# EI-CoreBioinformatics/portcullis

Measured on AMD Instinct MI355X. Metric: junc_reads_per_sec, higher is better.
Workload: dtype int32; 1 GPU; BASELINE configs[2]: synthetic 199999998 paired-end 150-bp reads, 25 contigs of GRCh38 lengths (3088286401 bp), 249999 junctions, orientation FR; reads_total=199999998, junctions_total=249999, contigs=25, reads_rank0=199999998, pairs_rank0=66692850

## Files before the change

### portcullis_amd/csrc/pjb_api.hip

```cpp
#include "pjb_host.hip.h"
#include "pjb_kernels.hip.h"

static int slot_init(pjb_ctx *c, int k);
static void aux_streams(pjb_ctx *c) {
    if (!c->stream3) (void)hipStreamCreateWithFlags(&c->stream3, hipStreamNonBlocking);
    if (!c->stream4) (void)hipStreamCreateWithFlags(&c->stream4, hipStreamNonBlocking);
}

extern "C" {

namespace {
std::mutex g_host_mu;
std::map<void *, size_t> g_host_registered;
}
void *pjb_host_alloc(size_t bytes) {
    if (bytes >= ((size_t)8 << 20)) {
        const size_t huge = (size_t)2 << 20, len = (bytes + huge - 1) & ~(huge - 1);
        void *p = mmap(nullptr, len, PROT_READ | PROT_WRITE, MAP_PRIVATE | MAP_ANONYMOUS, -1, 0);
        if (p != MAP_FAILED) {
            (void)madvise(p, len, MADV_HUGEPAGE);
            const size_t nt = std::min<size_t>(4, len >> 24);
            auto touch = [&](size_t t) {
                const size_t per = ((len / std::max<size_t>(nt, 1)) + huge - 1) & ~(huge - 1), a = std::min(len, per * t), b = std::min(len, a + per);
                for (size_t o = a; o < b; o += 4096) ((volatile uint8_t *)p)[o] = 0;
// ... 85 lines not shown
    hipDeviceProp_t prop;
    e = hipGetDeviceProperties(&prop, cfg->device);
    if (e != hipSuccess) return fail(nullptr, PJB_ERR_HIP, "hipGetDeviceProperties: %s", hipGetErrorString(e));
    cmark("hipSetDevice, hipGetDeviceProperties");
    const int n_cu = prop.multiProcessorCount;
    if (prop.warpSize != 64)
        return fail(nullptr, PJB_ERR_NO_DEVICE, "device %d (%s) is not a wave64 CDNA device", cfg->device, prop.gcnArchName);
    pjb_ctx *c = new (std::nothrow) pjb_ctx();
    if (!c) return fail(nullptr, PJB_ERR_NOMEM, "out of host memory");
    const int dev = cfg->device;
    auto attributes = [dev] {
        (void)hipSetDevice(dev);
        ingest_kernel_attributes();
        (void)hipFuncSetAttribute((const void *)rs_scatter<0, u64>, hipFuncAttributeMaxDynamicSharedMemorySize, (int)rs_scatter_lds_bytes(RS_MAX_BITS));
        (void)hipFuncSetAttribute((const void *)rs_scatter<0, u32>, hipFuncAttributeMaxDynamicSharedMemorySize, (int)rs_scatter_lds_bytes(RS_MAX_BITS, 4));
    };
    std::thread attr_thread(attributes);
    struct JoinAttr {
        std::thread &t;
        ~JoinAttr() {
            if (t.joinable()) t.join();
        }
    } join_attr{attr_thread};
    c->cfg = *cfg;
    memset(&c->timing, 0, sizeof c->timing);
    e = hipStreamCreateWithFlags(&c->stream, hipStreamNonBlocking);
    if (e != hipSuccess) {
        delete c;
        return fail(nullptr, PJB_ERR_HIP, "hipStreamCreate: %s", hipGetErrorString(e));
    }
// ... 706 lines not shown
        pass_bits.assign((size_t)n_pass, sort_bits / n_pass);
        for (int p = 0; p < sort_bits % n_pass; p++) pass_bits[(size_t)p]++;
        const int dbits = pass_bits[0];
        int rc2;
        if ((rc2 = ensure(c, S.hist, (size_t)plan_tiles * (1u << dbits) * 4))) return rc2;
        if ((rc2 = ensure(c, S.hist_scan, (size_t)plan_tiles * (1u << dbits) * 4))) return rc2;
        if ((rc2 = ensure(c, S.bintotal, (size_t)4 << dbits))) return rc2;
        if ((rc2 = ensure(c, S.hist_part, (size_t)((plan_tiles + RSP_TILES - 1) / RSP_TILES) * (1u << dbits) * 4))) return rc2;
        return PJB_OK;
    };
    const bool run_route = lim.dense && lim.run_sort;
    RunOut ro;
    memset(&ro, 0, sizeof ro);
    const u32 run_cap = (u32)std::min<u64>((u64)PL / 8 + 64ull * rs_tiles, 0xfff00000ull);
    const u32 ro_tiles = (run_cap + RS_TILE - 1) / RS_TILE;
    u64 *ro_total = nullptr, *ro_key[2] = {nullptr, nullptr};
    u32 *run_dest = nullptr, *ro_idx[2] = {nullptr, nullptr};
    if (run_route) {
        auto al = [](size_t b) { return (b + 255) & ~(size_t)255; };
        const size_t slack = (size_t)run_cap + RS_TILE;
        const size_t at_tf = 256, at_tn = at_tf + al((size_t)rs_tiles * 4), at_key = at_tn + al((size_t)rs_tiles * 4), at_cnt = at_key + al(slack * 8),
                     at_dest = at_cnt + al((size_t)run_cap * 4), at_k0 = at_dest + al((size_t)run_cap * 4), at_k1 = at_k0 + al(slack * 8),
                     at_i0 = at_k1 + al(slack * 8), at_i1 = at_i0 + al(slack * 4), at_end = at_i1 + al(slack * 4);
        if ((rc = ensure(c, S.runs, at_end))) return rc;
        uint8_t *b = (uint8_t *)S.runs.p;
        ro.n_runs = (u32 *)b;
        ro_total = (u64 *)(b + 8);
        ro.tile_first = (u32 *)(b + at_tf);
        ro.tile_n = (u32 *)(b + at_tn);
        ro.key = (u64 *)(b + at_key);
// ... 29 lines not shown
        if (run_route) plan_tiles = ro_tiles;
        if ((rc = plan_passes())) return rc;
        LAUNCH(c, "kd_assign", kd_assign, dim3(rs_tiles), dim3(256), okey, d_P, kf, (const u64 *)S.bitmap.p, (const u32 *)S.wrank.p,
               (const u32 *)S.ends.p, (const u32 *)S.firstid.p, JL, (const u64 *)S.total.p, (u32 *)S.jidbam.p, (u32 *)S.acc.p, (const u64 *)S.jkey.p,
               (const int32_t *)S.ancl.p, (const int32_t *)S.ancr.p, d_err, d_cs, run_route ? 0 : pass_bits[0], (u32 *)S.hist.p, ro);
        first_hist_done = !run_route;
        if ((rc = fork_k4b())) return rc;
        LAUNCH(c, "kd_reset", kd_reset, dim3(cand_blocks), dim3(256), (const u64 *)cand, (const u32 *)cand_rank, kf, JL, (const ContigStats *)d_cs,
               (u64 *)S.bitmap.p, (u32 *)S.ends.p, (u32 *)S.pagecnt.p);
        S.dense_at_rest = true;
    } else if ((rc = plan_passes()))
        return rc;
    int cur = 0, shift = 0;
    static const char *const rs_names[4] = {"rs_hist", "rs_panel_sums", "rs_panel_scan", "rs_scatter"};
    static const char *const ro_names[6] = {"ro_hist", "ro_panel_sums", "ro_panel_scan", "ro_scatter", "ro_offsets", "rs_place"};
    auto sort_pass = [&](auto key_tag, const void *kin_v, void *kout_v, const u32 *vin, u32 *vout, int bits, const u32 *d_n, u32 tiles,
                         const char *const *names) -> int {
        using K = decltype(key_tag);
        const K *kin = (const K *)kin_v;
        K *kout = (K *)kout_v;
        if (!(shift == 0 && first_hist_done))
            LAUNCH(c, names[0], rs_hist<K>, dim3(tiles), dim3(256), kin, d_n, shift, bits, (u32 *)S.hist.p, tiles);
        {
            const u32 nb = 1u << bits, n_panels = (tiles + RSP_TILES - 1) / RSP_TILES;
            LAUNCH(c, names[1], rs_panel_sums, dim3(n_panels, (nb + 255) / 256), dim3(256), (const u32 *)S.hist.p, tiles, nb, (u32 *)S.hist_part.p);
            LAUNCH(c, names[2], rs_panel_scan, dim3(n_panels, (nb + 255) / 256), dim3(256), (const u32 *)S.hist.p, (const u32 *)S.hist_part.p, tiles, nb,
                   (u32 *)S.hist_scan.p, (u32 *)S.bintotal.p);
        }
#define RS_SCATTER(B)                                                                                                                          \
    LAUNCH_LDS(c, names[3], (rs_scatter<B, K>), dim3(tiles), dim3(256), rs_scatter_lds_bytes(bits, sizeof(K)), kin, vin, kout, vout, d_n, \
               shift, bits, (const u32 *)S.hist_scan.p, (const u32 *)S.bintotal.p, tiles)
        switch (bits) {
        case 9: RS_SCATTER(9); break;
        case 10: RS_SCATTER(10); break;
        case 11: RS_SCATTER(11); break;
        default: RS_SCATTER(0); break;
        }
#undef RS_SCATTER
        return PJB_OK;
    };
    for (int p = 0; p < n_pass; p++) {
        const int bits = pass_bits[(size_t)p];
        if (bits <= 0) break;
        if (run_route) {
            rc = sort_pass((u64)0, p == 0 ? (const void *)ro.key : (const void *)ro_key[cur], ro_key[cur ^ 1], p == 0 ? nullptr : (const u32 *)ro_idx[cur],
                           ro_idx[cur ^ 1], bits, (const u32 *)ro.n_runs, ro_tiles, ro_names);
        } else {
            const u32 *vin = p == 0 ? nullptr : (const u32 *)S.idx[cur].p;
            u32 *vout = (u32 *)S.idx[cur ^ 1].p;
            if (lim.dense) rc = sort_pass((u32)0, p == 0 ? S.jidbam.p : S.key[cur].p, S.key[cur ^ 1].p, vin, vout, bits, d_P, rs_tiles, rs_names);
            else rc = sort_pass((u64)0, p == 0 ? S.okey.p : S.key[cur].p, S.key[cur ^ 1].p, vin, vout, bits, d_P, rs_tiles, rs_names);
        }
        if (rc) return rc;
        cur ^= 1;
        shift += bits;
    }
    if (run_route) {
        const u32 *order = ro_idx[cur];
        if ((rc = run_scan(c, ro_names[4], RunCountFn{(const u32 *)ro.cnt, order}, RunDestSink{run_dest, order}, (u64)run_cap, ro_total, (const u32 *)ro.n_runs)))
            return rc;
        cur = 1;
        LAUNCH(c, ro_names[5], rs_place, dim3(rs_tiles), dim3(256), (const u32 *)S.jidbam.p, d_P, (const u64 *)ro.key, (const u32 *)run_dest,
               (const u32 *)ro.tile_first, (const u32 *)ro.tile_n, run_cap, ro.tile_bits, (u32 *)S.key[cur].p, (u32 *)S.idx[cur].p);
        n_pass = 1;
    }
    f.n_pass = n_pass;
    const u32 *sidx = (const u32 *)S.idx[cur].p;
    f.sidx = sidx;
    const u32 *jid_sorted = lim.dense ? (const u32 *)S.key[cur].p : (const u32 *)S.jid.p;
    f.jid_sorted = jid_sorted;
    STAGE_EVENT(2);
    if ((rc = ensure(c, S.entsum, (size_t)JL * 8 + 16))) return rc;
    const u32 n_slices_lim = (PL + 63) / 64 + 1;
    const hipStream_t tl = st;
// ... 101 lines not shown
    }
    const hipStream_t rows_stream = c->side_stream ? c->stream3 : tl;
    if (rows_stream != tl) {
        HIP_TRY(c, hipEventRecord(S.ev_rows, tl));
        HIP_TRY(c, hipStreamWaitEvent(rows_stream, S.ev_rows, 0));
    }
    {
        struct StreamScope {
            pjb_ctx *c;
            hipStream_t main;
            ~StreamScope() { c->stream = main; }
        } scope{c, c->stream};
        c->stream = rows_stream;
        LAUNCH(c, "k6_rows_out", k6_rows_out, dim3(K6_BLOCKS), dim3(256), (const u64 *)S.rows.p, (const ContigStats *)d_cs,
               (u64 *)c->rows_table, row_base, mirror_base, (RowCursor *)c->b_cursor.p, mirror_table, mirror_room, d_err, d_gen_cnt, S.pub_dev,
               (const MemberStats *)d_members, d_member_junc, n_members);
    }
    S.at_rest = true;
    HIP_TRY(c, hipEventRecord(S.ev[7], rows_stream));
    HIP_TRY(c, hipEventRecord(S.ev_done, rows_stream));
#undef STAGE_EVENT
    f.queued = true;
    return PJB_OK;
}

static void wait_flight(pjb_ctx *c, Flight &f) {
    if (f.queued) (void)hipEventSynchronize(c->sl[f.slot].ev_done);
}

static void unqueue_followers(pjb_ctx *c) {
    for (int k = 1; k < c->n_fl; k++) {
// ... 277 lines not shown
            R.n_junctions = ms[m].n_junc;
            pairs += ms[m].n_pairs;
            juncs += ms[m].n_junc;
        }
        if (pairs != cs.n_pairs || juncs != J)
            return fail(c, PJB_ERR_STATE, "finish_group: members hold %llu pairs / %llu junctions, the chain %llu / %u", (unsigned long long)pairs,
                        (unsigned long long)juncs, (unsigned long long)cs.n_pairs, J);
        Rsum.spliced = cs.spliced;
        Rsum.unspliced = cs.unspliced;
        Rsum.sum_len = cs.sum_len;
        Rsum.min_len = cs.min_len;
        Rsum.max_len = cs.max_len;
    }
    c->junc_seen = std::max(c->junc_seen, group ? J / (u32)n_members : J);
    if (f.n_reads > 0) c->junc_per_read = std::max(c->junc_per_read, (double)J / (double)f.n_reads);
    c->timing.sort_passes = f.n_pass;
    c->timing.repeats = repeats;
    c->timing.repeat_reasons = repeat_reasons;
    c->timing.generic_pairs = 0;
    c->timing.generic_reads = 0;
    c->timing.checked_reads = *(const u32 *)(S.pub + PUB_CHECKED_AT);
    for (u32 k = 0; k < GEN_SHARDS; k++) {
        c->timing.generic_pairs += ((const u32 *)(S.pub + PUB_GEN_AT))[k];
        c->timing.generic_reads += ((const u32 *)(S.pub + PUB_GREADS_AT))[k];
    }
    c->timing.position_runs = cs.R;
    c->timing.candidates = lim.dense ? cs.n_cand : 0;
    const size_t old = c->rows_n;
    {
        u32 at[2];
// ... 275 lines not shown
}

int pjb_set_option(pjb_ctx *c, const char *name, int64_t value) {
    if (!c || !name) return PJB_ERR_ARG;
    if (c->n_fl) return fail(c, PJB_ERR_STATE, "set_option: target %d is still queued", c->fl[0].tid);
    const std::string n = name;
    if (n == "overlap") c->side_stream = value != 0;
    else if (n == "dense_ids") c->dense_ids = value != 0;
    else if (n == "extra_dense") c->extra_dense_only = value != 0;
    else if (n == "sort_floor") c->sort_floor = (u32)std::max<int64_t>(1, std::min<int64_t>(value, 1 << 30));
    else if (n == "window_skip") c->window_skip = value != 0;
    else if (n == "run_sort") c->run_sort = value != 0;
    else if (n == "run_window") {
        if (value < 0 || value > (int64_t)RUN_W) return fail(c, PJB_ERR_ARG, "set_option: run_window takes 0 (the default, %u) to %u", RUN_W, RUN_W);
        c->run_window = (u32)value;
    } else if (n == "grow_batch") {
        if (value < 0 || value > 32768) return fail(c, PJB_ERR_ARG, "set_option: grow_batch takes 0 (the default: what the pool holds) to 32768 trees");
        c->grow_batch = (u32)value;
    } else if (n == "knn_chunk") {
        if (value < 0 || value > (1 << 22)) return fail(c, PJB_ERR_ARG, "set_option: knn_chunk takes 0 (the default: sized to fill the chip) to %d base rows", 1 << 22);
        c->knn_chunk = (u32)value;
    } else if (n == "list_cap") c->list_cap_forced = (u32)std::max<int64_t>(0, std::min<int64_t>(value, 1 << 30));
    else return fail(c, PJB_ERR_ARG, "set_option: unknown option '%s'", name);
    return PJB_OK;
}

int pjb_get_timing(const pjb_ctx *c, pjb_timing *out) {
    if (!c || !out) return PJB_ERR_ARG;
    if (c->cfg.abi_version >= 4) *out = c->timing;
    else memcpy(out, &c->timing, offsetof(pjb_timing, repeats));
// ... 5 lines not shown
```

### portcullis_amd/csrc/pjb_device.hip.h

```cpp
#pragma once

#include <hip/hip_runtime.h>
#include <stdint.h>

#include "../../include/portcullis_amd.h"

namespace pjb {

typedef unsigned long long u64;
typedef unsigned int u32;

struct DevBatch {
    const int32_t *pos;
    const uint16_t *flag;
    const uint8_t *mapq;
    const uint8_t *xs;
    const int32_t *l_qseq;
    const int32_t *mtid;
    const int32_t *mpos;
    const uint32_t *cig_off;
    const uint32_t *cigar;
    const uint32_t *seq_off;
    const uint8_t *seq4;
    const u64 *name_hash;
// ... 437 lines not shown
    __syncthreads();
    u64 run = s_pref[0] + s_pref[1] + s_pref[2] + s_pref[3];
    if (blockIdx.x == n_tiles - 1 && threadIdx.x == 0) *total = run + tile_sums[blockIdx.x];
    const u64 base = (u64)blockIdx.x * SCAN_TILE;
#pragma unroll
    for (int k = 0; k < 8; k++) {
        u64 i = base + (u64)k * 256 + threadIdx.x;
        u64 v = i < n ? f(i) : 0;
        u64 tot;
        u64 ex = block_escan_256<u64>(v, sm, &tot);
        if (i < n) g(i, v, run + ex);
        run += tot;
    }
}

struct ArrU32Fn {
    const u32 *a;
    __device__ u64 operator()(u64 i) const { return a[i]; }
};
struct ArrU8Fn {
    const uint8_t *a;
    __device__ u64 operator()(u64 i) const { return a[i]; }
};
struct ArrI32Fn {
    const int32_t *a;
    __device__ u64 operator()(u64 i) const { return (u64)(int64_t)a[i]; }
};
struct ExclusiveU32Sink {
    u32 *out;
    __device__ void operator()(u64 i, u64, u64 ex) const { out[i] = (u32)ex; }
// ... 70 lines not shown
    case 'W': return 'S';
    case 'X': return 'X';
    case 'Y': return 'R';
    default: return 0;
    }
}

__device__ __forceinline__ void fetch_clamp(int32_t glen, int32_t &b, int32_t &e) {
    if (e < b) b = e;
    if (b < 0) b = 0;
    else if (glen <= b) b = glen - 1;
    if (e < 0) e = 0;
    else if (glen <= e) e = glen - 1;
}

constexpr int PUB_BASE_AT = 240, PUB_ERR_AT = 256, PUB_XCNT_AT = 320 , PUB_CHECKED_AT = 384 , PUB_GEN_AT = 512, PUB_MEMBERS_AT = 1536, PUB_GREADS_AT = 3072, PUB_BYTES = 4096;
static_assert(PUB_MEMBERS_AT + GROUP_MAX * sizeof(MemberStats) <= PUB_BYTES && sizeof(MemberStats) % 8 == 0, "control block layout");

}
```

### portcullis_amd/csrc/pjb_host.hip.h

```cpp
#pragma once
#include "pjb_device.hip.h"
#include "pjb_extra_types.hip.h"

#include <algorithm>
#include <sys/mman.h>
#include <thread>
#include <chrono>
#include <cstdarg>
#include <cstdio>
#include <cstdlib>
#include <cstring>
#include <map>
#include <memory>
#include <mutex>
#include <string>
#include <thread>
#include <vector>

using namespace pjb;


inline thread_local std::string g_create_error;
inline thread_local std::string g_thread_error;
inline thread_local const void *g_thread_error_ctx = nullptr;
// ... 214 lines not shown
    std::vector<void *> graveyard;
    std::mutex grave_mu;
    size_t last_rows_n = 0;
    uint8_t *mirror = nullptr;
    size_t mirror_cap = 0;
    int64_t *mirror_hdr = nullptr;
    size_t mirror_rows = 0;
    int64_t mirror_acc[5] = {0, 0, 0, INT32_MAX, 0};
    pjb_timing timing;
    int radix_max_bits = 11;
    double junc_per_read = 0;
    u32 sort_floor = 1u << 16;
    bool window_skip = true;
    bool run_sort = true;
    u32 run_window = 0;
    u32 list_cap_forced = 0;
    bool k1_serial = true;
    hipEvent_t last_k1_ev = nullptr;
    int k1s_blocks_forced = 0;
    bool ktime = false;
    std::vector<std::string> knames;
    std::vector<int64_t> kcount;
    std::vector<double> kms;
    std::vector<std::string> ktime_only;
    Buf *scan_tiles = nullptr;
    Buf b_scan_tiles;
    Buf b_inf_comp, b_inf_out, b_inf_blocks, b_inf_status, b_inf_scratch, b_inf_bitmap;
    Buf b_dfl_in, b_dfl_sym, b_dfl_slots, b_dfl_size, b_dfl_off, b_dfl_packed;
    Buf b_bam_seg, b_bam_rec, b_bam_ctl;
    struct IndexState *index = nullptr;
// ... 239 lines not shown
    Buf &tiles = c->scan_tiles ? *c->scan_tiles : c->b_scan_tiles;
    int rc = ensure(c, tiles, (size_t)nt * 8);
    if (rc) return rc;
    u64 *ts = (u64 *)tiles.p;
    std::string t = tag;
    LAUNCH(c, (t + "_reduce").c_str(), (scan_reduce_kernel<F>), dim3(nt), dim3(256), f, n, ts, d_n);
    if (nt <= SCAN2_MAX_TILES) {
        LAUNCH(c, (t + "_apply").c_str(), (scan_apply2_kernel<F, G>), dim3(nt), dim3(256), f, g, n, (const u64 *)ts, d_n, d_total);
        return PJB_OK;
    }
    LAUNCH(c, (t + "_tiles").c_str(), scan_tiles_kernel, dim3(1), dim3(1024), ts, nt, d_total);
    LAUNCH(c, (t + "_apply").c_str(), (scan_apply_kernel<F, G>), dim3(nt), dim3(256), f, g, n, (const u64 *)ts, d_n);
    return PJB_OK;
}

inline void *slab_alloc(pjb_ctx *c, OpenContig &oc, size_t bytes) {
    bytes = (std::max<size_t>(bytes, 16) + 255) & ~(size_t)255;
    for (auto &s : oc.slabs)
        if (s.cap - s.used >= bytes) {
            void *r = s.p + s.used;
            s.used += bytes;
            return r;
        }
    {
        const size_t want = oc.slabs.empty() ? std::max(bytes, oc.slab_hint) : bytes;
        long best = -1;
        for (size_t k = 0; k < c->slab_pool.size(); k++)
            if (c->slab_pool[k].cap >= want && (best < 0 || c->slab_pool[k].cap < c->slab_pool[(size_t)best].cap)) best = (long)k;
        if (best >= 0) {
            Slab s = c->slab_pool[(size_t)best];
// ... 84 lines not shown
```

### portcullis_amd/csrc/pjb_kernels.hip.h

```cpp
#pragma once

#include "pjb_device.hip.h"

namespace pjb {

__global__ __launch_bounds__(256) void k0_upper(uint8_t *g, int64_t n, int do_upper, int *has_x) {
    int64_t i = ((int64_t)blockIdx.x * 256 + threadIdx.x) * 16;
    bool x = false;
    for (int64_t j = i; j < n && j < i + 16; j++) {
        uint8_t c = g[j];
        x |= (c == 'X' || (do_upper && c == 'x'));
    }
    if (__ballot(x) && lane_id() == 0) atomicOr(has_x, 1);
    if (!do_upper) return;
    if (i + 16 <= n && ((uintptr_t)(g + i) & 15) == 0) {
        uint4 v = *reinterpret_cast<uint4 *>(g + i);
        u32 *w = reinterpret_cast<u32 *>(&v);
#pragma unroll
        for (int k = 0; k < 4; k++) {
            u32 x = w[k], r = 0;
#pragma unroll
            for (int b = 0; b < 4; b++) {
                u32 c = (x >> (8 * b)) & 0xff;
                if (c >= 'a' && c <= 'z') c -= 32;
// ... 2152 lines not shown
__device__ __forceinline__ void wave_hist_add(u32 *h, u32 d, bool valid) {
    u64 rem = __ballot(valid);
    const int lane = lane_id();
#pragma unroll
    for (int it = 0; it < 2; it++) {
        if (rem == 0) return;
        const int first = __ffsll((long long)rem) - 1;
        const u32 d0 = __shfl(d, first, 64);
        const u64 m = __ballot(valid && d == d0) & rem;
        if (lane == first) atomicAdd(&h[d0], (u32)__popcll(m));
        rem &= ~m;
    }
    if ((rem >> lane) & 1ull) atomicAdd(&h[d], 1u);
}

template <typename K>
__global__ __launch_bounds__(256) void rs_hist(const K *keys, const u32 *np, int shift, int bits, u32 *hist, u32 n_tiles) {
    __shared__ u32 h[RS_MAX_BINS];
    const u32 n = *np;
    const u32 nb = 1u << bits;
    for (u32 d = threadIdx.x; d < nb; d += 256) h[d] = 0;
    __syncthreads();
    const u32 base = blockIdx.x * RS_TILE;
    const u32 mask = nb - 1;
    K kk[RS_ITEMS];
#pragma unroll
    for (int k = 0; k < RS_ITEMS; k++) {
        const u32 i = base + k * 256 + threadIdx.x;
        kk[k] = i < n ? keys[i] : (K)0;
    }
#pragma unroll
    for (int k = 0; k < RS_ITEMS; k++) {
        const u32 i = base + k * 256 + threadIdx.x;
        wave_hist_add(h, (u32)(kk[k] >> shift) & mask, i < n);
    }
    __syncthreads();
    for (u32 d = threadIdx.x; d < nb; d += 256) hist[(size_t)blockIdx.x * nb + d] = h[d];
}

constexpr u32 RSP_TILES = 64;
__global__ __launch_bounds__(256) void rs_panel_sums(const u32 *hist, u32 n_tiles, u32 nb, u32 *psum) {
    const u32 d = blockIdx.y * 256 + threadIdx.x;
    if (d >= nb) return;
    const u32 t0 = blockIdx.x * RSP_TILES, t1 = t0 + RSP_TILES < n_tiles ? t0 + RSP_TILES : n_tiles;
    u32 sum = 0;
    for (u32 t = t0; t < t1; t += 8) {
        u32 v[8];
#pragma unroll
        for (int k = 0; k < 8; k++) v[k] = t + k < t1 ? hist[(size_t)(t + k) * nb + d] : 0u;
#pragma unroll
        for (int k = 0; k < 8; k++) sum += v[k];
    }
// ... 11 lines not shown
#pragma unroll
        for (int k = 0; k < 8; k++) run += v[k];
    }
    const u32 t0 = panel * RSP_TILES, t1 = t0 + RSP_TILES < n_tiles ? t0 + RSP_TILES : n_tiles;
    for (u32 t = t0; t < t1; t += 8) {
        u32 v[8];
#pragma unroll
        for (int k = 0; k < 8; k++) v[k] = t + k < t1 ? hist[(size_t)(t + k) * nb + d] : 0u;
#pragma unroll
        for (int k = 0; k < 8; k++) {
            if (t + k < t1) hist_scan[(size_t)(t + k) * nb + d] = run;
            run += v[k];
        }
    }
    if (t1 == n_tiles) row_total[d] = run;
}

__host__ __device__ constexpr size_t rs_scatter_lds_bytes(int bits, size_t key_bytes = 8) {
    return (size_t)RS_TILE * key_bytes + ((size_t)4 << bits) + ((size_t)8 << bits);
}
constexpr int RS_PF = 2;

template <int BITS>
__device__ __forceinline__ u64 wave_match_digit(u32 d, bool valid, int bits) {
    u64 peers = __ballot(valid);
    u32 lo = (u32)peers, hi = (u32)(peers >> 32);
    auto step = [&](int bit) {
        const int m = __builtin_amdgcn_sbfe((int)d, bit, 1);
        const u64 bb = __ballot(m != 0);
        lo &= ~((u32)bb ^ (u32)m);
        hi &= ~((u32)(bb >> 32) ^ (u32)m);
    };
    if constexpr (BITS > 0) {
#pragma unroll
        for (int bit = 0; bit < BITS; bit++) step(bit);
    } else {
        for (int bit = 0; bit < bits; bit++) step(bit);
    }
    return ((u64)hi << 32) | lo;
}

template <int BITS, typename K>
__global__ __launch_bounds__(256, 3) void rs_scatter(const K *kin, const u32 *vin, K *kout, u32 *vout, const u32 *np, int shift,
                                                      int bits, const u32 *hist_scan, const u32 *row_total, u32 n_tiles) {
    extern __shared__ __attribute__((aligned(16))) unsigned char rs_smem[];
    __shared__ u64 s_scan[4];
    const u32 n = *np;
    if ((u64)blockIdx.x * RS_TILE >= n) return;
    if (BITS > 0) bits = BITS;
    const u32 nb = 1u << bits;
    const u32 mask = nb - 1;
    K *kbuf = (K *)rs_smem;
    u32 *ibuf = (u32 *)rs_smem;
    u32 *delta = (u32 *)(rs_smem + (size_t)RS_TILE * sizeof(K));
    unsigned short *wcnt = (unsigned short *)(delta + nb);
    for (u32 d = threadIdx.x; d < 2 * nb; d += 256) ((u32 *)wcnt)[d] = 0;
    __syncthreads();
    const u32 tile = blockIdx.x;
    const int w = __builtin_amdgcn_readfirstlane(threadIdx.x >> 6), lane = lane_id();
    unsigned short *wc = wcnt + (size_t)w * nb;
    const u32 base = tile * RS_TILE + w * (RS_TILE / 4);
    const u64 lt = (1ull << lane) - 1;
    K key[RS_ITEMS];
    u32 val[RS_ITEMS];
    u32 rkp[RS_ITEMS / 2];
    const K *kp = kin + base;
#pragma unroll
    for (int r = 0; r < RS_ITEMS; r++) key[r] = kp[r * 64 + lane];
    const u32 per = (nb + 255) / 256;
    const u32 d0 = threadIdx.x * per;
    u32 pf_rt[RS_PF], pf_hs[RS_PF];
#pragma unroll
    for (int k = 0; k < RS_PF; k++) {
        const u32 d = d0 + k;
        const bool on = (u32)k < per && d < nb;
        pf_rt[k] = on ? row_total[d] : 0u;
        pf_hs[k] = on ? hist_scan[(size_t)tile * nb + d] : 0u;
    }
#pragma unroll
    for (int r = 0; r < RS_ITEMS; r++) {
        const u32 i = base + r * 64 + lane;
        const bool valid = i < n;
        const u32 d = (u32)(key[r] >> shift) & mask;
        const u64 peers = wave_match_digit<BITS>(d, valid, bits);
        const u32 lower = (u32)__popcll(peers & lt), group = (u32)__popcll(peers);
        const int leader = valid ? __ffsll((long long)peers) - 1 : lane;
        u32 before = 0;
        if (valid && lane == leader) {
            before = wc[d];
            wc[d] = (unsigned short)(before + group);
        }
        const u32 rank = __shfl(before, leader, 64) + lower;
        rkp[r >> 1] = (r & 1) ? (rkp[r >> 1] | (rank << 16)) : rank;
    }
    if (vin) {
        const u32 *vp = vin + base;
#pragma unroll
        for (int r = 0; r < RS_ITEMS; r++) val[r] = vp[r * 64 + lane];
    } else {
#pragma unroll
        for (int r = 0; r < RS_ITEMS; r++) val[r] = base + r * 64 + lane;
    }
    __syncthreads();
    u32 mine = 0, below = 0;
    for (u32 k = 0; k < per; k++) {
        const u32 d = d0 + k;
        if (d < nb) {
            mine += (u32)wcnt[d] + wcnt[nb + d] + wcnt[2 * nb + d] + wcnt[3 * nb + d];
            below += k < RS_PF ? pf_rt[k < RS_PF ? k : 0] : row_total[d];
        }
    }
    u64 tot;
    const u64 both = block_escan_256<u64>((u64)mine | ((u64)below << 32), s_scan, &tot);
    u32 tstart = (u32)both, dbase = (u32)(both >> 32);
    for (u32 k = 0; k < per; k++) {
        const u32 d = d0 + k;
        if (d >= nb) break;
        const u32 c0 = wcnt[d], c1 = wcnt[nb + d], c2 = wcnt[2 * nb + d], c3 = wcnt[3 * nb + d];
        const u32 gfirst = dbase + (k < RS_PF ? pf_hs[k < RS_PF ? k : 0] : hist_scan[(size_t)tile * nb + d]);
        dbase += k < RS_PF ? pf_rt[k < RS_PF ? k : 0] : row_total[d];
        delta[d] = gfirst - tstart;
        wcnt[d] = (unsigned short)tstart;
        wcnt[nb + d] = (unsigned short)(tstart + c0);
        wcnt[2 * nb + d] = (unsigned short)(tstart + c0 + c1);
        wcnt[3 * nb + d] = (unsigned short)(tstart + c0 + c1 + c2);
        tstart += c0 + c1 + c2 + c3;
    }
    __syncthreads();
#pragma unroll
    for (int r = 0; r < RS_ITEMS; r++) {
        const u32 i = base + r * 64 + lane;
        const u32 lp = ((rkp[r >> 1] >> ((r & 1) * 16)) & 0xffffu) + wc[(u32)(key[r] >> shift) & mask];
        rkp[r >> 1] = (r & 1) ? ((rkp[r >> 1] & 0xffffu) | (lp << 16)) : ((rkp[r >> 1] & 0xffff0000u) | lp);
        if (i < n) kbuf[lp] = key[r];
    }
    __syncthreads();
    const u32 cnt = min((u32)RS_TILE, n - tile * RS_TILE);
    u32 digp[RS_ITEMS / 2];
#pragma unroll
    for (int r = 0; r < RS_ITEMS; r++) {
        const u32 j = r * 256 + threadIdx.x;
        const K kk = j < cnt ? kbuf[j] : (K)0;
        const u32 d = (u32)(kk >> shift) & mask;
        digp[r >> 1] = (r & 1) ? (digp[r >> 1] | (d << 16)) : d;
        if (j < cnt) kout[delta[d] + j] = kk;
    }
    __syncthreads();
#pragma unroll
    for (int r = 0; r < RS_ITEMS; r++) {
        const u32 i = base + r * 64 + lane;
        if (i < n) ibuf[(rkp[r >> 1] >> ((r & 1) * 16)) & 0xffffu] = val[r];
    }
    __syncthreads();
#pragma unroll
    for (int r = 0; r < RS_ITEMS; r++) {
        const u32 j = r * 256 + threadIdx.x;
        if (j < cnt) vout[delta[(digp[r >> 1] >> ((r & 1) * 16)) & 0xffffu] + j] = ibuf[j];
    }
}

struct RunCountFn {
    const u32 *cnt, *order;
    __device__ u64 operator()(u64 i) const { return cnt[order[i]]; }
};
struct RunDestSink {
    u32 *dest;
    const u32 *order;
    __device__ void operator()(u64 i, u64, u64 ex) const { dest[order[i]] = (u32)ex; }
};
__global__ __launch_bounds__(256) void rs_place(const u32 *jid_bam, const u32 *np, const u64 *run_key, const u32 *run_dest, const u32 *tile_first,
                                                const u32 *tile_n, u32 run_cap, int tile_bits, u32 *kout, u32 *vout) {
    __shared__ u32 s_dest[RUN_W];
// ... 871 lines not shown
        }
        R.hamming5p = h5;
        R.hamming3p = h3;
    }
    rows[j] = R;
}

constexpr int ROW_U64 = (int)(sizeof(pjb_junction_row) / 8);
static_assert(sizeof(pjb_junction_row) % 8 == 0, "rows are copied in 8-byte units");
struct RowCursor {
    u32 rows, mirror_rows;
    u32 blocks_done;
    u32 _pad;
};
__device__ __forceinline__ void publish_chain(const ContigStats *cs, u64 *err, u32 *gen_cnt, uint8_t *host, int64_t base, int64_t mirror_base,
                                              RowCursor *cur, const MemberStats *members, u32 *member_junc, int n_members);
__global__ __launch_bounds__(256) void k6_rows_out(const u64 *rows, const ContigStats *cs, u64 *host_table, int64_t base, int64_t mirror_base,
                                                   RowCursor *cur, u64 *mirror_table, u32 mirror_room, u64 *err, u32 *gen_cnt, uint8_t *host_pub,
                                                   const MemberStats *members, u32 *member_junc, int n_members) {
    const u32 nj = cs->J;
    const u64 n = (u64)nj * ROW_U64;
    const u64 at = base >= 0 ? (u64)base : (u64)cur->rows;
    const u64 mat = mirror_base >= 0 ? (u64)mirror_base : (u64)cur->mirror_rows;
    const bool to_mirror = mirror_table && mat + nj <= (u64)mirror_room;
    for (u64 i = (u64)blockIdx.x * 256 + threadIdx.x; i < n; i += (u64)gridDim.x * 256) {
        const u64 v = rows[i];
        host_table[at * ROW_U64 + i] = v;
        if (to_mirror) mirror_table[mat * ROW_U64 + i] = v;
    }
    __shared__ u32 s_last;
    __threadfence_system();
    __syncthreads();
    if (threadIdx.x == 0) s_last = atomicAdd(&cur->blocks_done, 1u) + 1u == gridDim.x ? 1u : 0u;
    __syncthreads();
    if (!s_last) return;
    __threadfence_system();
    if (threadIdx.x == 0) cur->blocks_done = 0;
    publish_chain(cs, err, gen_cnt, host_pub, base, mirror_base, cur, members, member_junc, n_members);
}

__device__ __forceinline__ void publish_chain(const ContigStats *cs, u64 *err, u32 *gen_cnt, uint8_t *host, int64_t base, int64_t mirror_base,
                                              RowCursor *cur, const MemberStats *members, u32 *member_junc, int n_members) {
    const u32 t = threadIdx.x;
    if (n_members > 1 && t < (u32)n_members) {
        MemberStats S = members[t];
        S.n_junc = member_junc[t];
        reinterpret_cast<MemberStats *>(host + PUB_MEMBERS_AT)[t] = S;
    }
    static_assert(sizeof(ContigStats) % 8 == 0 && sizeof(ContigStats) <= PUB_BASE_AT, "control block layout");
    static_assert(PUB_GEN_AT + GEN_SHARDS * 4 <= PUB_MEMBERS_AT && PUB_MEMBERS_AT + GROUP_MAX * sizeof(MemberStats) <= PUB_GREADS_AT &&
                      PUB_GREADS_AT + GEN_SHARDS * 4 <= PUB_BYTES,
                  "control block layout");
    if (t < sizeof(ContigStats) / 8) reinterpret_cast<u64 *>(host)[t] = reinterpret_cast<const u64 *>(cs)[t];
    __shared__ u32 s_chk[4];
    {
        const u32 chk = wave_total<DppAdd>(t < GEN_SHARDS ? gen_cnt[t * GEN_CNT_STRIDE + 2] : 0u);
        if (lane_id() == 0) s_chk[t >> 6] = chk;
    }
    if (t < GEN_SHARDS) {
        reinterpret_cast<u32 *>(host + PUB_GEN_AT)[t] = gen_cnt[t * GEN_CNT_STRIDE + 1];
        reinterpret_cast<u32 *>(host + PUB_GREADS_AT)[t] = gen_cnt[t * GEN_CNT_STRIDE];
        reinterpret_cast<uint4 *>(gen_cnt + t * GEN_CNT_STRIDE)[0] = make_uint4(0, 0, 0, 0);
        reinterpret_cast<uint4 *>(gen_cnt + t * GEN_CNT_STRIDE)[1] = make_uint4(0, 0, 0, 0);
    }
    if (t == 0) {
        *reinterpret_cast<u64 *>(host + PUB_ERR_AT) = *err;
        *err = ~0ull;
        const u32 at = base >= 0 ? (u32)base : cur->rows, mat = mirror_base >= 0 ? (u32)mirror_base : cur->mirror_rows;
        reinterpret_cast<u32 *>(host + PUB_BASE_AT)[0] = at;
        reinterpret_cast<u32 *>(host + PUB_BASE_AT)[1] = mat;
        cur->rows = at + cs->J;
        cur->mirror_rows = mat + cs->J;
    }
    __syncthreads();
    if (t < (u32)GROUP_MAX) member_junc[t] = 0;
    if (t == 0) *reinterpret_cast<u32 *>(host + PUB_CHECKED_AT) = s_chk[0] + s_chk[1] + s_chk[2] + s_chk[3];
}

}
```

Before: 30.16 billion reads/s.

## Size run-list radix sort grids from observed run counts with persistent strided kernels

Result: no change. 30.21 billion reads/s (median of 2 runs) (+0.2%).

```diff
diff --git a/portcullis_amd/csrc/pjb_api.hip b/portcullis_amd/csrc/pjb_api.hip
--- a/portcullis_amd/csrc/pjb_api.hip
+++ b/portcullis_amd/csrc/pjb_api.hip
@@ -123,6 +123,7 @@
         ingest_kernel_attributes();
         (void)hipFuncSetAttribute((const void *)rs_scatter<0, u64>, hipFuncAttributeMaxDynamicSharedMemorySize, (int)rs_scatter_lds_bytes(RS_MAX_BITS));
         (void)hipFuncSetAttribute((const void *)rs_scatter<0, u32>, hipFuncAttributeMaxDynamicSharedMemorySize, (int)rs_scatter_lds_bytes(RS_MAX_BITS, 4));
+        (void)hipFuncSetAttribute((const void *)rs_scatter<0, u64, true>, hipFuncAttributeMaxDynamicSharedMemorySize, (int)rs_scatter_lds_bytes(RS_MAX_BITS));
     };
     std::thread attr_thread(attributes);
     struct JoinAttr {
@@ -859,6 +860,8 @@
     memset(&ro, 0, sizeof ro);
     const u32 run_cap = (u32)std::min<u64>((u64)PL / 8 + 64ull * rs_tiles, 0xfff00000ull);
     const u32 ro_tiles = (run_cap + RS_TILE - 1) / RS_TILE;
+    const u32 ro_grid = c->run_grid ? std::min(c->run_grid, ro_tiles)
+                                    : std::min(ro_tiles, c->run_chains_seen ? std::max<u32>(32, 2 * c->run_tiles_seen) : 256u);
     u64 *ro_total = nullptr, *ro_key[2] = {nullptr, nullptr};
     u32 *run_dest = nullptr, *ro_idx[2] = {nullptr, nullptr};
     if (run_route) {
@@ -918,15 +921,31 @@
     int cur = 0, shift = 0;
     static const char *const rs_names[4] = {"rs_hist", "rs_panel_sums", "rs_panel_scan", "rs_scatter"};
     static const char *const ro_names[6] = {"ro_hist", "ro_panel_sums", "ro_panel_scan", "ro_scatter", "ro_offsets", "rs_place"};
-    auto sort_pass = [&](auto key_tag, const void *kin_v, void *kout_v, const u32 *vin, u32 *vout, int bits, const u32 *d_n, u32 tiles,
+    auto sort_pass = [&](auto key_tag, auto list_tag, const void *kin_v, void *kout_v, const u32 *vin, u32 *vout, int bits, const u32 *d_n, u32 tiles,
                          const char *const *names) -> int {
         using K = decltype(key_tag);
         const K *kin = (const K *)kin_v;
         K *kout = (K *)kout_v;
+        const u32 nb = 1u << bits, n_panels = (tiles + RSP_TILES - 1) / RSP_TILES;
+        if constexpr (decltype(list_tag)::value) {
+            LAUNCH(c, names[0], (rs_hist<K, true>), dim3(ro_grid), dim3(256), kin, d_n, shift, bits, (u32 *)S.hist.p, tiles);
+            LAUNCH(c, names[2], rl_digit_scan, dim3((nb + 255) / 256), dim3(256), (const u32 *)S.hist.p, d_n, tiles, nb, (u32 *)S.hist_scan.p,
+                   (u32 *)S.bintotal.p);
+#define RL_SCATTER(B)                                                                                                                       \
+    LAUNCH_LDS(c, names[3], (rs_scatter<B, u64, true>), dim3(ro_grid), dim3(256), rs_scatter_lds_bytes(bits, sizeof(K)), kin, vin, kout, vout, d_n, \
+               shift, bits, (const u32 *)S.hist_scan.p, (const u32 *)S.bintotal.p, tiles)
+            switch (bits) {
+            case 9: RL_SCATTER(9); break;
+            case 10: RL_SCATTER(10); break;
+            case 11: RL_SCATTER(11); break;
+            default: RL_SCATTER(0); break;
+            }
+#undef RL_SCATTER
+            return PJB_OK;
+        }
         if (!(shift == 0 && first_hist_done))
             LAUNCH(c, names[0], rs_hist<K>, dim3(tiles), dim3(256), kin, d_n, shift, bits, (u32 *)S.hist.p, tiles);
         {
-            const u32 nb = 1u << bits, n_panels = (tiles + RSP_TILES - 1) / RSP_TILES;
             LAUNCH(c, names[1], rs_panel_sums, dim3(n_panels, (nb + 255) / 256), dim3(256), (const u32 *)S.hist.p, tiles, nb, (u32 *)S.hist_part.p);
             LAUNCH(c, names[2], rs_panel_scan, dim3(n_panels, (nb + 255) / 256), dim3(256), (const u32 *)S.hist.p, (const u32 *)S.hist_part.p, tiles, nb,
                    (u32 *)S.hist_scan.p, (u32 *)S.bintotal.p);
@@ -947,13 +966,13 @@
         const int bits = pass_bits[(size_t)p];
         if (bits <= 0) break;
         if (run_route) {
-            rc = sort_pass((u64)0, p == 0 ? (const void *)ro.key : (const void *)ro_key[cur], ro_key[cur ^ 1], p == 0 ? nullptr : (const u32 *)ro_idx[cur],
+            rc = sort_pass((u64)0, std::true_type{}, p == 0 ? (const void *)ro.key : (const void *)ro_key[cur], ro_key[cur ^ 1], p == 0 ? nullptr : (const u32 *)ro_idx[cur],
                            ro_idx[cur ^ 1], bits, (const u32 *)ro.n_runs, ro_tiles, ro_names);
         } else {
             const u32 *vin = p == 0 ? nullptr : (const u32 *)S.idx[cur].p;
             u32 *vout = (u32 *)S.idx[cur ^ 1].p;
-            if (lim.dense) rc = sort_pass((u32)0, p == 0 ? S.jidbam.p : S.key[cur].p, S.key[cur ^ 1].p, vin, vout, bits, d_P, rs_tiles, rs_names);
-            else rc = sort_pass((u64)0, p == 0 ? S.okey.p : S.key[cur].p, S.key[cur ^ 1].p, vin, vout, bits, d_P, rs_tiles, rs_names);
+            if (lim.dense) rc = sort_pass((u32)0, std::false_type{}, p == 0 ? S.jidbam.p : S.key[cur].p, S.key[cur ^ 1].p, vin, vout, bits, d_P, rs_tiles, rs_names);
+            else rc = sort_pass((u64)0, std::false_type{}, p == 0 ? S.okey.p : S.key[cur].p, S.key[cur ^ 1].p, vin, vout, bits, d_P, rs_tiles, rs_names);
         }
         if (rc) return rc;
         cur ^= 1;
@@ -961,7 +980,9 @@
     }
     if (run_route) {
         const u32 *order = ro_idx[cur];
-        if ((rc = run_scan(c, ro_names[4], RunCountFn{(const u32 *)ro.cnt, order}, RunDestSink{run_dest, order}, (u64)run_cap, ro_total, (const u32 *)ro.n_runs)))
+        const u32 scan_grid = c->run_grid ? c->run_grid : 2 * ro_grid;
+        if ((rc = run_scan_strided(c, ro_names[4], RunCountFn{(const u32 *)ro.cnt, order}, RunDestSink{run_dest, order}, (u64)run_cap, ro_total,
+                                   (const u32 *)ro.n_runs, scan_grid)))
             return rc;
         cur = 1;
         LAUNCH(c, ro_names[5], rs_place, dim3(rs_tiles), dim3(256), (const u32 *)S.jidbam.p, d_P, (const u64 *)ro.key, (const u32 *)run_dest,
@@ -1093,7 +1114,7 @@
         c->stream = rows_stream;
         LAUNCH(c, "k6_rows_out", k6_rows_out, dim3(K6_BLOCKS), dim3(256), (const u64 *)S.rows.p, (const ContigStats *)d_cs,
                (u64 *)c->rows_table, row_base, mirror_base, (RowCursor *)c->b_cursor.p, mirror_table, mirror_room, d_err, d_gen_cnt, S.pub_dev,
-               (const MemberStats *)d_members, d_member_junc, n_members);
+               (const MemberStats *)d_members, d_member_junc, n_members, run_route ? (const u32 *)ro.n_runs : nullptr);
     }
     S.at_rest = true;
     HIP_TRY(c, hipEventRecord(S.ev[7], rows_stream));
@@ -1401,6 +1422,8 @@
     }
     c->junc_seen = std::max(c->junc_seen, group ? J / (u32)n_members : J);
     if (f.n_reads > 0) c->junc_per_read = std::max(c->junc_per_read, (double)J / (double)f.n_reads);
+    c->run_tiles_seen = std::max(c->run_tiles_seen, (*(const u32 *)(S.pub + PUB_RUNS_AT) + (u32)RS_TILE - 1) / (u32)RS_TILE);
+    c->run_chains_seen = true;
     c->timing.sort_passes = f.n_pass;
     c->timing.repeats = repeats;
     c->timing.repeat_reasons = repeat_reasons;
@@ -1706,6 +1729,9 @@
     else if (n == "run_window") {
         if (value < 0 || value > (int64_t)RUN_W) return fail(c, PJB_ERR_ARG, "set_option: run_window takes 0 (the default, %u) to %u", RUN_W, RUN_W);
         c->run_window = (u32)value;
+    } else if (n == "run_grid") {
+        if (value < 0 || value > 65536) return fail(c, PJB_ERR_ARG, "set_option: run_grid takes 0 (the default: a grid from the lists met so far) to 65536 blocks");
+        c->run_grid = (u32)value;
     } else if (n == "grow_batch") {
         if (value < 0 || value > 32768) return fail(c, PJB_ERR_ARG, "set_option: grow_batch takes 0 (the default: what the pool holds) to 32768 trees");
         c->grow_batch = (u32)value;
diff --git a/portcullis_amd/csrc/pjb_device.hip.h b/portcullis_amd/csrc/pjb_device.hip.h
--- a/portcullis_amd/csrc/pjb_device.hip.h
+++ b/portcullis_amd/csrc/pjb_device.hip.h
@@ -475,6 +475,60 @@
     }
 }
 
+template <typename F>
+__global__ __launch_bounds__(256) void scan_reduce_strided_kernel(F f, u64 n, u64 *tile_sums, const u32 *np) {
+    __shared__ u64 sm[4];
+    {
+        const u64 d = *np;
+        n = d < n ? d : n;
+    }
+    const u64 n_tiles = n == 0 ? 1 : (n + SCAN_TILE - 1) / SCAN_TILE;
+    for (u64 tile = blockIdx.x; tile < n_tiles; tile += gridDim.x) {
+        const u64 base = tile * SCAN_TILE;
+        u64 s = 0;
+#pragma unroll
+        for (int k = 0; k < 8; k++) {
+            u64 i = base + (u64)k * 256 + threadIdx.x;
+            if (i < n) s += f(i);
+        }
+        s = wave_sum(s);
+        if (lane_id() == 0) sm[threadIdx.x >> 6] = s;
+        __syncthreads();
+        if (threadIdx.x == 0) tile_sums[tile] = sm[0] + sm[1] + sm[2] + sm[3];
+        __syncthreads();
+    }
+}
+template <typename F, typename G>
+__global__ __launch_bounds__(256) void scan_apply2_strided_kernel(F f, G g, u64 n, const u64 *tile_sums, const u32 *np, u64 *total) {
+    __shared__ u64 sm[4];
+    __shared__ u64 s_pref[4];
+    {
+        const u64 d = *np;
+        n = d < n ? d : n;
+    }
+    const u64 n_tiles = n == 0 ? 1 : (n + SCAN_TILE - 1) / SCAN_TILE;
+    for (u64 tile = blockIdx.x; tile < n_tiles; tile += gridDim.x) {
+        u64 acc = 0;
+        for (u64 t = threadIdx.x; t < tile; t += 256) acc += tile_sums[t];
+        acc = wave_sum(acc);
+        if (lane_id() == 0) s_pref[threadIdx.x >> 6] = acc;
+        __syncthreads();
+        u64 run = s_pref[0] + s_pref[1] + s_pref[2] + s_pref[3];
+        if (tile == n_tiles - 1 && threadIdx.x == 0) *total = run + tile_sums[tile];
+        const u64 base = tile * SCAN_TILE;
+#pragma unroll
+        for (int k = 0; k < 8; k++) {
+            u64 i = base + (u64)k * 256 + threadIdx.x;
+            u64 v = i < n ? f(i) : 0;
+            u64 tot;
+            u64 ex = block_escan_256<u64>(v, sm, &tot);
+            if (i < n) g(i, v, run + ex);
+            run += tot;
+        }
+        __syncthreads();
+    }
+}
+
 struct ArrU32Fn {
     const u32 *a;
     __device__ u64 operator()(u64 i) const { return a[i]; }
@@ -575,7 +629,7 @@
     else if (glen <= e) e = glen - 1;
 }
 
-constexpr int PUB_BASE_AT = 240, PUB_ERR_AT = 256, PUB_XCNT_AT = 320 , PUB_CHECKED_AT = 384 , PUB_GEN_AT = 512, PUB_MEMBERS_AT = 1536, PUB_GREADS_AT = 3072, PUB_BYTES = 4096;
+constexpr int PUB_BASE_AT = 240, PUB_ERR_AT = 256, PUB_XCNT_AT = 320 , PUB_CHECKED_AT = 384 , PUB_RUNS_AT = 392 , PUB_GEN_AT = 512, PUB_MEMBERS_AT = 1536, PUB_GREADS_AT = 3072, PUB_BYTES = 4096;
 static_assert(PUB_MEMBERS_AT + GROUP_MAX * sizeof(MemberStats) <= PUB_BYTES && sizeof(MemberStats) % 8 == 0, "control block layout");
 
 }
diff --git a/portcullis_amd/csrc/pjb_host.hip.h b/portcullis_amd/csrc/pjb_host.hip.h
--- a/portcullis_amd/csrc/pjb_host.hip.h
+++ b/portcullis_amd/csrc/pjb_host.hip.h
@@ -252,6 +252,9 @@
     bool window_skip = true;
     bool run_sort = true;
     u32 run_window = 0;
+    u32 run_grid = 0;
+    u32 run_tiles_seen = 0;
+    bool run_chains_seen = false;
     u32 list_cap_forced = 0;
     bool k1_serial = true;
     hipEvent_t last_k1_ev = nullptr;
@@ -521,6 +524,21 @@
     return PJB_OK;
 }
 
+template <typename F, typename G>
+inline int run_scan_strided(pjb_ctx *c, const char *tag, F f, G g, u64 n, u64 *d_total, const u32 *d_n, u32 grid) {
+    const u32 nt = std::max<u32>(1, (u32)((n + SCAN_TILE - 1) / SCAN_TILE));
+    if (nt > SCAN2_MAX_TILES) return run_scan(c, tag, f, g, n, d_total, d_n);
+    Buf &tiles = c->scan_tiles ? *c->scan_tiles : c->b_scan_tiles;
+    int rc = ensure(c, tiles, (size_t)nt * 8);
+    if (rc) return rc;
+    u64 *ts = (u64 *)tiles.p;
+    grid = std::max<u32>(1, std::min(grid, nt));
+    std::string t = tag;
+    LAUNCH(c, (t + "_reduce").c_str(), (scan_reduce_strided_kernel<F>), dim3(grid), dim3(256), f, n, ts, d_n);
+    LAUNCH(c, (t + "_apply").c_str(), (scan_apply2_strided_kernel<F, G>), dim3(grid), dim3(256), f, g, n, (const u64 *)ts, d_n, d_total);
+    return PJB_OK;
+}
+
 inline void *slab_alloc(pjb_ctx *c, OpenContig &oc, size_t bytes) {
     bytes = (std::max<size_t>(bytes, 16) + 255) & ~(size_t)255;
     for (auto &s : oc.slabs)
diff --git a/portcullis_amd/csrc/pjb_kernels.hip.h b/portcullis_amd/csrc/pjb_kernels.hip.h
--- a/portcullis_amd/csrc/pjb_kernels.hip.h
+++ b/portcullis_amd/csrc/pjb_kernels.hip.h
@@ -2190,28 +2190,39 @@
     if ((rem >> lane) & 1ull) atomicAdd(&h[d], 1u);
 }
 
-template <typename K>
+__device__ __forceinline__ u32 rl_tiles(const u32 *np, u32 n_tiles) {
+    const u32 n = *np;
+    const u32 t = n / RS_TILE + (n % RS_TILE ? 1u : 0u);
+    return t < n_tiles ? t : n_tiles;
+}
+template <typename K, bool LIST = false>
 __global__ __launch_bounds__(256) void rs_hist(const K *keys, const u32 *np, int shift, int bits, u32 *hist, u32 n_tiles) {
     __shared__ u32 h[RS_MAX_BINS];
     const u32 n = *np;
     const u32 nb = 1u << bits;
-    for (u32 d = threadIdx.x; d < nb; d += 256) h[d] = 0;
-    __syncthreads();
-    const u32 base = blockIdx.x * RS_TILE;
     const u32 mask = nb - 1;
-    K kk[RS_ITEMS];
-#pragma unroll
-    for (int k = 0; k < RS_ITEMS; k++) {
-        const u32 i = base + k * 256 + threadIdx.x;
-        kk[k] = i < n ? keys[i] : (K)0;
-    }
-#pragma unroll
-    for (int k = 0; k < RS_ITEMS; k++) {
-        const u32 i = base + k * 256 + threadIdx.x;
-        wave_hist_add(h, (u32)(kk[k] >> shift) & mask, i < n);
-    }
-    __syncthreads();
-    for (u32 d = threadIdx.x; d < nb; d += 256) hist[(size_t)blockIdx.x * nb + d] = h[d];
+    for (u32 tile = blockIdx.x;; tile += gridDim.x) {
+        if constexpr (LIST)
+            if (tile >= rl_tiles(np, n_tiles)) break;
+        for (u32 d = threadIdx.x; d < nb; d += 256) h[d] = 0;
+        __syncthreads();
+        const u32 base = tile * RS_TILE;
+        K kk[RS_ITEMS];
+    #pragma unroll
+        for (int k = 0; k < RS_ITEMS; k++) {
+            const u32 i = base + k * 256 + threadIdx.x;
+            kk[k] = i < n ? keys[i] : (K)0;
+        }
+    #pragma unroll
+        for (int k = 0; k < RS_ITEMS; k++) {
+            const u32 i = base + k * 256 + threadIdx.x;
+            wave_hist_add(h, (u32)(kk[k] >> shift) & mask, i < n);
+        }
+        __syncthreads();
+        for (u32 d = threadIdx.x; d < nb; d += 256) hist[(size_t)tile * nb + d] = h[d];
+        if constexpr (!LIST) break;
+        __syncthreads();
+    }
 }
 
 constexpr u32 RSP_TILES = 64;
@@ -2253,6 +2264,24 @@
         }
     }
     if (t1 == n_tiles) row_total[d] = run;
+}
+
+__global__ __launch_bounds__(256) void rl_digit_scan(const u32 *hist, const u32 *np, u32 n_tiles, u32 nb, u32 *hist_scan, u32 *row_total) {
+    const u32 d = blockIdx.x * 256 + threadIdx.x;
+    if (d >= nb) return;
+    const u32 nt = rl_tiles(np, n_tiles);
+    u32 run = 0;
+    for (u32 t = 0; t < nt; t += 8) {
+        u32 v[8];
+#pragma unroll
+        for (int k = 0; k < 8; k++) v[k] = t + k < nt ? hist[(size_t)(t + k) * nb + d] : 0u;
+#pragma unroll
+        for (int k = 0; k < 8; k++) {
+            if (t + k < nt) hist_scan[(size_t)(t + k) * nb + d] = run;
+            run += v[k];
+        }
+    }
+    row_total[d] = run;
 }
 
 __host__ __device__ constexpr size_t rs_scatter_lds_bytes(int bits, size_t key_bytes = 8) {
@@ -2279,13 +2308,14 @@
     return ((u64)hi << 32) | lo;
 }
 
-template <int BITS, typename K>
-__global__ __launch_bounds__(256, 3) void rs_scatter(const K *kin, const u32 *vin, K *kout, u32 *vout, const u32 *np, int shift,
-                                                      int bits, const u32 *hist_scan, const u32 *row_total, u32 n_tiles) {
+template <int BITS, typename K, bool LIST = false>
+__global__ __launch_bounds__(256, LIST ? 1 : 3) void rs_scatter(const K *kin, const u32 *vin, K *kout, u32 *vout, const u32 *np, int shift,
+                                                                 int bits, const u32 *hist_scan, const u32 *row_total, u32 n_tiles) {
     extern __shared__ __attribute__((aligned(16))) unsigned char rs_smem[];
     __shared__ u64 s_scan[4];
     const u32 n = *np;
-    if ((u64)blockIdx.x * RS_TILE >= n) return;
+    if constexpr (!LIST)
+        if ((u64)blockIdx.x * RS_TILE >= n) return;
     if (BITS > 0) bits = BITS;
     const u32 nb = 1u << bits;
     const u32 mask = nb - 1;
@@ -2293,108 +2323,113 @@
     u32 *ibuf = (u32 *)rs_smem;
     u32 *delta = (u32 *)(rs_smem + (size_t)RS_TILE * sizeof(K));
     unsigned short *wcnt = (unsigned short *)(delta + nb);
-    for (u32 d = threadIdx.x; d < 2 * nb; d += 256) ((u32 *)wcnt)[d] = 0;
-    __syncthreads();
-    const u32 tile = blockIdx.x;
-    const int w = __builtin_amdgcn_readfirstlane(threadIdx.x >> 6), lane = lane_id();
-    unsigned short *wc = wcnt + (size_t)w * nb;
-    const u32 base = tile * RS_TILE + w * (RS_TILE / 4);
-    const u64 lt = (1ull << lane) - 1;
-    K key[RS_ITEMS];
-    u32 val[RS_ITEMS];
-    u32 rkp[RS_ITEMS / 2];
-    const K *kp = kin + base;
-#pragma unroll
-    for (int r = 0; r < RS_ITEMS; r++) key[r] = kp[r * 64 + lane];
-    const u32 per = (nb + 255) / 256;
-    const u32 d0 = threadIdx.x * per;
-    u32 pf_rt[RS_PF], pf_hs[RS_PF];
-#pragma unroll
-    for (int k = 0; k < RS_PF; k++) {
-        const u32 d = d0 + k;
-        const bool on = (u32)k < per && d < nb;
-        pf_rt[k] = on ? row_total[d] : 0u;
-        pf_hs[k] = on ? hist_scan[(size_t)tile * nb + d] : 0u;
-    }
-#pragma unroll
-    for (int r = 0; r < RS_ITEMS; r++) {
-        const u32 i = base + r * 64 + lane;
-        const bool valid = i < n;
-        const u32 d = (u32)(key[r] >> shift) & mask;
-        const u64 peers = wave_match_digit<BITS>(d, valid, bits);
-        const u32 lower = (u32)__popcll(peers & lt), group = (u32)__popcll(peers);
-        const int leader = valid ? __ffsll((long long)peers) - 1 : lane;
-        u32 before = 0;
-        if (valid && lane == leader) {
-            before = wc[d];
-            wc[d] = (unsigned short)(before + group);
-        }
-        const u32 rank = __shfl(before, leader, 64) + lower;
-        rkp[r >> 1] = (r & 1) ? (rkp[r >> 1] | (rank << 16)) : rank;
-    }
-    if (vin) {
-        const u32 *vp = vin + base;
-#pragma unroll
-        for (int r = 0; r < RS_ITEMS; r++) val[r] = vp[r * 64 + lane];
-    } else {
-#pragma unroll
-        for (int r = 0; r < RS_ITEMS; r++) val[r] = base + r * 64 + lane;
-    }
-    __syncthreads();
-    u32 mine = 0, below = 0;
-    for (u32 k = 0; k < per; k++) {
-        const u32 d = d0 + k;
-        if (d < nb) {
-            mine += (u32)wcnt[d] + wcnt[nb + d] + wcnt[2 * nb + d] + wcnt[3 * nb + d];
-            below += k < RS_PF ? pf_rt[k < RS_PF ? k : 0] : row_total[d];
-        }
-    }
-    u64 tot;
-    const u64 both = block_escan_256<u64>((u64)mine | ((u64)below << 32), s_scan, &tot);
-    u32 tstart = (u32)both, dbase = (u32)(both >> 32);
-    for (u32 k = 0; k < per; k++) {
-        const u32 d = d0 + k;
-        if (d >= nb) break;
-        const u32 c0 = wcnt[d], c1 = wcnt[nb + d], c2 = wcnt[2 * nb + d], c3 = wcnt[3 * nb + d];
-        const u32 gfirst = dbase + (k < RS_PF ? pf_hs[k < RS_PF ? k : 0] : hist_scan[(size_t)tile * nb + d]);
-        dbase += k < RS_PF ? pf_rt[k < RS_PF ? k : 0] : row_total[d];
-        delta[d] = gfirst - tstart;
-        wcnt[d] = (unsigned short)tstart;
-        wcnt[nb + d] = (unsigned short)(tstart + c0);
-        wcnt[2 * nb + d] = (unsigned short)(tstart + c0 + c1);
-        wcnt[3 * nb + d] = (unsigned short)(tstart + c0 + c1 + c2);
-        tstart += c0 + c1 + c2 + c3;
-    }
-    __syncthreads();
-#pragma unroll
-    for (int r = 0; r < RS_ITEMS; r++) {
-        const u32 i = base + r * 64 + lane;
-        const u32 lp = ((rkp[r >> 1] >> ((r & 1) * 16)) & 0xffffu) + wc[(u32)(key[r] >> shift) & mask];
-        rkp[r >> 1] = (r & 1) ? ((rkp[r >> 1] & 0xffffu) | (lp << 16)) : ((rkp[r >> 1] & 0xffff0000u) | lp);
-        if (i < n) kbuf[lp] = key[r];
-    }
-    __syncthreads();
-    const u32 cnt = min((u32)RS_TILE, n - tile * RS_TILE);
-    u32 digp[RS_ITEMS / 2];
-#pragma unroll
-    for (int r = 0; r < RS_ITEMS; r++) {
-        const u32 j = r * 256 + threadIdx.x;
-        const K kk = j < cnt ? kbuf[j] : (K)0;
-        const u32 d = (u32)(kk >> shift) & mask;
-        digp[r >> 1] = (r & 1) ? (digp[r >> 1] | (d << 16)) : d;
-        if (j < cnt) kout[delta[d] + j] = kk;
-    }
-    __syncthreads();
-#pragma unroll
-    for (int r = 0; r < RS_ITEMS; r++) {
-        const u32 i = base + r * 64 + lane;
-        if (i < n) ibuf[(rkp[r >> 1] >> ((r & 1) * 16)) & 0xffffu] = val[r];
-    }
-    __syncthreads();
-#pragma unroll
-    for (int r = 0; r < RS_ITEMS; r++) {
-        const u32 j = r * 256 + threadIdx.x;
-        if (j < cnt) vout[delta[(digp[r >> 1] >> ((r & 1) * 16)) & 0xffffu] + j] = ibuf[j];
+    for (u32 tile = blockIdx.x;; tile += gridDim.x) {
+        if constexpr (LIST)
+            if (tile >= rl_tiles(np, n_tiles)) break;
+        for (u32 d = threadIdx.x; d < 2 * nb; d += 256) ((u32 *)wcnt)[d] = 0;
+        __syncthreads();
+        const int w = __builtin_amdgcn_readfirstlane(threadIdx.x >> 6), lane = lane_id();
+        unsigned short *wc = wcnt + (size_t)w * nb;
+        const u32 base = tile * RS_TILE + w * (RS_TILE / 4);
+        const u64 lt = (1ull << lane) - 1;
+        K key[RS_ITEMS];
+        u32 val[RS_ITEMS];
+        u32 rkp[RS_ITEMS / 2];
+        const K *kp = kin + base;
+    #pragma unroll
+        for (int r = 0; r < RS_ITEMS; r++) key[r] = kp[r * 64 + lane];
+        const u32 per = (nb + 255) / 256;
+        const u32 d0 = threadIdx.x * per;
+        u32 pf_rt[RS_PF], pf_hs[RS_PF];
+    #pragma unroll
+        for (int k = 0; k < RS_PF; k++) {
+            const u32 d = d0 + k;
+            const bool on = (u32)k < per && d < nb;
+            pf_rt[k] = on ? row_total[d] : 0u;
+            pf_hs[k] = on ? hist_scan[(size_t)tile * nb + d] : 0u;
+        }
+    #pragma unroll
+        for (int r = 0; r < RS_ITEMS; r++) {
+            const u32 i = base + r * 64 + lane;
+            const bool valid = i < n;
+            const u32 d = (u32)(key[r] >> shift) & mask;
+            const u64 peers = wave_match_digit<BITS>(d, valid, bits);
+            const u32 lower = (u32)__popcll(peers & lt), group = (u32)__popcll(peers);
+            const int leader = valid ? __ffsll((long long)peers) - 1 : lane;
+            u32 before = 0;
+            if (valid && lane == leader) {
+                before = wc[d];
+                wc[d] = (unsigned short)(before + group);
+            }
+            const u32 rank = __shfl(before, leader, 64) + lower;
+            rkp[r >> 1] = (r & 1) ? (rkp[r >> 1] | (rank << 16)) : rank;
+        }
+        if (vin) {
+            const u32 *vp = vin + base;
+    #pragma unroll
+            for (int r = 0; r < RS_ITEMS; r++) val[r] = vp[r * 64 + lane];
+        } else {
+    #pragma unroll
+            for (int r = 0; r < RS_ITEMS; r++) val[r] = base + r * 64 + lane;
+        }
+        __syncthreads();
+        u32 mine = 0, below = 0;
+        for (u32 k = 0; k < per; k++) {
+            const u32 d = d0 + k;
+            if (d < nb) {
+                mine += (u32)wcnt[d] + wcnt[nb + d] + wcnt[2 * nb + d] + wcnt[3 * nb + d];
+                below += k < RS_PF ? pf_rt[k < RS_PF ? k : 0] : row_total[d];
+            }
+        }
+        u64 tot;
+        const u64 both = block_escan_256<u64>((u64)mine | ((u64)below << 32), s_scan, &tot);
+        u32 tstart = (u32)both, dbase = (u32)(both >> 32);
+        for (u32 k = 0; k < per; k++) {
+            const u32 d = d0 + k;
+            if (d >= nb) break;
+            const u32 c0 = wcnt[d], c1 = wcnt[nb + d], c2 = wcnt[2 * nb + d], c3 = wcnt[3 * nb + d];
+            const u32 gfirst = dbase + (k < RS_PF ? pf_hs[k < RS_PF ? k : 0] : hist_scan[(size_t)tile * nb + d]);
+            dbase += k < RS_PF ? pf_rt[k < RS_PF ? k : 0] : row_total[d];
+            delta[d] = gfirst - tstart;
+            wcnt[d] = (unsigned short)tstart;
+            wcnt[nb + d] = (unsigned short)(tstart + c0);
+            wcnt[2 * nb + d] = (unsigned short)(tstart + c0 + c1);
+            wcnt[3 * nb + d] = (unsigned short)(tstart + c0 + c1 + c2);
+            tstart += c0 + c1 + c2 + c3;
+        }
+        __syncthreads();
+    #pragma unroll
+        for (int r = 0; r < RS_ITEMS; r++) {
+            const u32 i = base + r * 64 + lane;
+            const u32 lp = ((rkp[r >> 1] >> ((r & 1) * 16)) & 0xffffu) + wc[(u32)(key[r] >> shift) & mask];
+            rkp[r >> 1] = (r & 1) ? ((rkp[r >> 1] & 0xffffu) | (lp << 16)) : ((rkp[r >> 1] & 0xffff0000u) | lp);
+            if (i < n) kbuf[lp] = key[r];
+        }
+        __syncthreads();
+        const u32 cnt = min((u32)RS_TILE, n - tile * RS_TILE);
+        u32 digp[RS_ITEMS / 2];
+    #pragma unroll
+        for (int r = 0; r < RS_ITEMS; r++) {
+            const u32 j = r * 256 + threadIdx.x;
+            const K kk = j < cnt ? kbuf[j] : (K)0;
+            const u32 d = (u32)(kk >> shift) & mask;
+            digp[r >> 1] = (r & 1) ? (digp[r >> 1] | (d << 16)) : d;
+            if (j < cnt) kout[delta[d] + j] = kk;
+        }
+        __syncthreads();
+    #pragma unroll
+        for (int r = 0; r < RS_ITEMS; r++) {
+            const u32 i = base + r * 64 + lane;
+            if (i < n) ibuf[(rkp[r >> 1] >> ((r & 1) * 16)) & 0xffffu] = val[r];
+        }
+        __syncthreads();
+    #pragma unroll
+        for (int r = 0; r < RS_ITEMS; r++) {
+            const u32 j = r * 256 + threadIdx.x;
+            if (j < cnt) vout[delta[(digp[r >> 1] >> ((r & 1) * 16)) & 0xffffu] + j] = ibuf[j];
+        }
+        if constexpr (!LIST) break;
+        __syncthreads();
     }
 }
 
@@ -3296,10 +3331,10 @@
     u32 _pad;
 };
 __device__ __forceinline__ void publish_chain(const ContigStats *cs, u64 *err, u32 *gen_cnt, uint8_t *host, int64_t base, int64_t mirror_base,
-                                              RowCursor *cur, const MemberStats *members, u32 *member_junc, int n_members);
+                                              RowCursor *cur, const MemberStats *members, u32 *member_junc, int n_members, const u32 *n_runs);
 __global__ __launch_bounds__(256) void k6_rows_out(const u64 *rows, const ContigStats *cs, u64 *host_table, int64_t base, int64_t mirror_base,
                                                    RowCursor *cur, u64 *mirror_table, u32 mirror_room, u64 *err, u32 *gen_cnt, uint8_t *host_pub,
-                                                   const MemberStats *members, u32 *member_junc, int n_members) {
+                                                   const MemberStats *members, u32 *member_junc, int n_members, const u32 *n_runs) {
     const u32 nj = cs->J;
     const u64 n = (u64)nj * ROW_U64;
     const u64 at = base >= 0 ? (u64)base : (u64)cur->rows;
@@ -3318,11 +3353,11 @@
     if (!s_last) return;
     __threadfence_system();
     if (threadIdx.x == 0) cur->blocks_done = 0;
-    publish_chain(cs, err, gen_cnt, host_pub, base, mirror_base, cur, members, member_junc, n_members);
+    publish_chain(cs, err, gen_cnt, host_pub, base, mirror_base, cur, members, member_junc, n_members, n_runs);
 }
 
 __device__ __forceinline__ void publish_chain(const ContigStats *cs, u64 *err, u32 *gen_cnt, uint8_t *host, int64_t base, int64_t mirror_base,
-                                              RowCursor *cur, const MemberStats *members, u32 *member_junc, int n_members) {
+                                              RowCursor *cur, const MemberStats *members, u32 *member_junc, int n_members, const u32 *n_runs) {
     const u32 t = threadIdx.x;
     if (n_members > 1 && t < (u32)n_members) {
         MemberStats S = members[t];
@@ -3353,6 +3388,7 @@
         reinterpret_cast<u32 *>(host + PUB_BASE_AT)[1] = mat;
         cur->rows = at + cs->J;
         cur->mirror_rows = mat + cs->J;
+        *reinterpret_cast<u32 *>(host + PUB_RUNS_AT) = n_runs ? *n_runs : 0u;
     }
     __syncthreads();
     if (t < (u32)GROUP_MAX) member_junc[t] = 0;
```
